# endernewton/tf-faster-rcnn

Measured on NVIDIA H100. Metric: images/sec, higher is better.
Workload: dtype f16x3 (fp32-grade: fp16 hi/lo split of both operands, 3 wgmma f16 MMAs per product, fp32 accumulate)

## Files before the change

### include/frcnn_b200.h

```cpp
#ifndef FRCNN_B200_H_
#define FRCNN_B200_H_

#include <stddef.h>
#include <stdint.h>

#ifdef __cplusplus
extern "C" {
#endif

typedef enum {
  FRCNN_OK = 0,
  FRCNN_ERR_CUDA = -1,
  FRCNN_ERR_ARG = -2,
  FRCNN_ERR_NO_DEVICE = -3,
  FRCNN_ERR_DRIVER_ENTRY = -4,
  FRCNN_ERR_CAPACITY = -5
} frcnn_status;

#define FRCNN_NMS_PLUS_ONE 1u
#define FRCNN_NMS_INCLUSIVE 2u
#define FRCNN_NMS_SKIP_DEGENERATE 4u
#define FRCNN_NMS_MODE_CPU_NMS (FRCNN_NMS_PLUS_ONE | FRCNN_NMS_INCLUSIVE)
#define FRCNN_NMS_MODE_GPU_NMS (FRCNN_NMS_PLUS_ONE)
#define FRCNN_NMS_MODE_TF (FRCNN_NMS_SKIP_DEGENERATE)

#define FRCNN_ACT_NONE 0
#define FRCNN_ACT_RELU 1
#define FRCNN_ACT_RELU6 2

int frcnn_version(void);
int frcnn_last_error(char* buf, size_t buflen);
int frcnn_check_device(int device_id);
int frcnn_zero_async(void* dev_ptr, size_t bytes, void* stream);

typedef struct frcnn_graph frcnn_graph;
int frcnn_graph_begin(void* stream);
int frcnn_graph_end(void* stream, frcnn_graph** out);
int frcnn_graph_launch(const frcnn_graph* g, void* stream);
void frcnn_graph_destroy(frcnn_graph* g);

int frcnn_nms_host(int* keep_out, int* num_out, const float* boxes_host, int boxes_num, int boxes_dim,
                   float nms_overlap_thresh, int device_id, unsigned flags);

int frcnn_nms_sorted_dev(const float* boxes_dev, int n, float thresh, unsigned flags, int max_out,
                         int* keep_dev, int* num_dev, void* stream);

typedef struct frcnn_conv_plan frcnn_conv_plan;
#define FRCNN_CONV_F16X3 0
#define FRCNN_CONV_TF32X3 1
#define FRCNN_CONV_F16X1 2

typedef struct {
  const float* in_dev;
  const void* w_hi_dev;
  const void* w_lo_dev;
  const float* scale_dev;
  const float* shift_dev;
  const float* residual_dev;
  float* out_dev;
  int n, h, w, cin;
  int cout, kh, kw, stride;
  int pad_t, pad_l;
  int ho, wo;
  int act;
  int block_n;
  int kb_per_chunk;
  int split_k;
  int impl;
  float out_mult;
  const float* in2_dev;
  int cin2;
  float* mean_dev;
  int mean_hw;
} frcnn_conv_desc;

int frcnn_conv_plan_create(frcnn_conv_plan** out, const frcnn_conv_desc* d);
int frcnn_conv_plan_run(const frcnn_conv_plan* p, void* stream);
int frcnn_conv_plan_geometry(const frcnn_conv_desc* d, int sm_count, int* out16);
int frcnn_conv_plan_info(const frcnn_conv_plan* p, int* block_n, int* tile_n, int* tile_h, int* tile_w,
                         int* grid_m, int* grid_n, int* splits, int* smem_bytes);
int frcnn_conv_plan_set_trace(frcnn_conv_plan* p, long long* trace_dev);
void frcnn_conv_plan_destroy(frcnn_conv_plan* p);
int frcnn_debug_watchdog(unsigned int* out16, int reset);

int frcnn_pack_conv_weights(const float* w_hwio_dev, void* w_hi_dev, void* w_lo_dev, int kh, int kw,
                            int cin, int cout, int wexp, void* stream);
int frcnn_pack_conv_weights_tf32(const float* w_hwio_dev, float* w_hi_dev, float* w_lo_dev, int kh, int kw,
                                 int cin, int cout, void* stream);

int frcnn_conv_first(const float* in_dev, const float* w_hwio_dev, const float* scale_dev,
                     const float* shift_dev, float* out_dev, int n, int h, int w, int cout, int k,
                     int stride, int pad_t, int pad_l, int ho, int wo, int act, void* stream);
int frcnn_depthwise3x3(const float* in_dev, const float* w_dev, const float* scale_dev,
                       const float* shift_dev, float* out_dev, int n, int h, int w, int c, int stride,
                       int pad_t, int pad_l, int ho, int wo, int act, void* stream);
int frcnn_max_pool(const float* in_dev, float* out_dev, int n, int h, int w, int c, int k, int stride,
                   int pad_t, int pad_l, int ho, int wo, int pad_is_neg_inf, void* stream);
int frcnn_spatial_mean(const float* in_dev, float* out_dev, int r, int hw, int c, void* stream);

int frcnn_preprocess(const unsigned char* img_dev, int h0, int w0, const double* means3, double fx, double fy,
                     float* blob_dev, int H, int W, void* stream);
int frcnn_preprocess_hflip(const unsigned char* img_dev, int h0, int w0, const double* means3, double fx, double fy,
                           float* blob_dev, int H, int W, void* stream);


int frcnn_rpn_decode(const float* rpn_out_dev, int ld, int delta_col, const float* base_anchors_dev, int num_anchors,
                     int batch, int fh, int fw, int feat_stride, float im_h, float im_w, float* scores_dev,
                     float* props_dev, void* stream);
size_t frcnn_sort_workspace_bytes(int n);
int frcnn_sort_desc(const float* keys_dev, int n, int batch, int* order_dev, float* sorted_keys_dev, void* workspace_dev,
                    size_t workspace_bytes, void* stream);
int frcnn_proposals(const float* props_dev, const float* scores_dev, const int* order_dev, int n, int batch,
                    int pre_nms_top_n, int post_nms_top_n, float thresh, unsigned flags, float* rois_dev,
                    float* roi_scores_dev, int* keep_dev, int* num_dev, void* stream);
int frcnn_crop_pool(const float* feat_dev, int batch, int fh, int fw, int c, const float* rois_dev, int r, int pooled,
                    int pre_pool, float* out_dev, void* stream);
#define FRCNN_ROI_ALIGN_MAX_SAMPLING 16
int frcnn_roi_align(const float* feat_dev, int batch, int fh, int fw, int c, const float* rois_dev, int r, int pooled,
                    float spatial_scale, int sampling_ratio, int aligned, float* out_dev, void* stream);
int frcnn_roi_pool(const float* feat_dev, int batch, int fh, int fw, int c, const float* rois_dev, int r, int pooled,
                   float spatial_scale, float* out_dev, void* stream);
int frcnn_cls_finish(const float* head_out_dev, int ld, int r, int num_classes, const float* stds4,
                     const float* means4, float* cls_score_dev, float* cls_prob_dev, float* bbox_pred_dev,
                     void* stream);
int frcnn_bbox_decode(const float* rois_dev, const float* bbox_pred_dev, int r, int num_classes, int batch,
                      const float* im_meta_dev, float* pred_boxes_dev, void* stream);
size_t frcnn_detect_post_workspace_bytes(int r, int num_classes, int batch);
int frcnn_detect_post(const float* cls_prob_dev, const float* pred_boxes_dev, const int* num_rois_dev, int r, int batch,
                      int num_classes, float score_thresh, float nms_thresh, unsigned flags,
                      int max_per_image, int max_det, float* det_dev, int* ndet_dev, int record_stride, int* keep_dev,
                      int* keep_cnt_dev, float* keep_score_dev, void* workspace_dev, size_t workspace_bytes, void* stream);
#define FRCNN_SOFT_NMS_LINEAR 0
#define FRCNN_SOFT_NMS_GAUSSIAN 1
#define FRCNN_SOFT_NMS_HARD 2
int frcnn_soft_nms_host(float* dets_out, int* keep_out, int* num_out, const float* dets_host, int n, int dim, int method,
                        float sigma, float nt, float score_thresh, int device_id);
int frcnn_detect_post_soft(const float* cls_prob_dev, const float* pred_boxes_dev, const int* num_rois_dev, int r, int batch,
                           int num_classes, float score_thresh, int method, float sigma, float nt, float prune_thresh,
                           int max_per_image, int max_det, float* det_dev, int* ndet_dev, int record_stride, int* keep_dev,
                           int* keep_cnt_dev, float* keep_score_dev, void* workspace_dev, size_t workspace_bytes, void* stream);
#define FRCNN_BOX_VOTE_ID 0
#define FRCNN_BOX_VOTE_AVG 1
#define FRCNN_BOX_VOTE_IOU_AVG 2
#define FRCNN_BOX_VOTE_GENERALIZED_AVG 3
#define FRCNN_BOX_VOTE_QUASI_SUM 4
#define FRCNN_BOX_VOTE_TEMP_AVG 5
int frcnn_box_vote_host(float* dets_out, const float* top_host, int n_top, int top_dim, const float* all_host, int n_all,
                        int all_dim, float thresh, int method, float beta, int device_id);
int frcnn_detect_post_vote(const float* cls_prob_dev, const float* pred_boxes_dev, const int* num_rois_dev, int r, int batch,
                           int num_classes, float score_thresh, float nms_thresh, unsigned flags, int max_per_image, int max_det,
                           float* det_dev, int* ndet_dev, int record_stride, int* keep_dev, int* keep_cnt_dev, float* keep_score_dev,
                           void* workspace_dev, size_t workspace_bytes, float vote_thresh, int vote_method, float vote_beta,
                           float* vote_box_dev, void* stream);
int frcnn_detect_post_soft_vote(const float* cls_prob_dev, const float* pred_boxes_dev, const int* num_rois_dev, int r, int batch,
                                int num_classes, float score_thresh, int method, float sigma, float nt, float prune_thresh,
                                int max_per_image, int max_det, float* det_dev, int* ndet_dev, int record_stride, int* keep_dev,
                                int* keep_cnt_dev, float* keep_score_dev, void* workspace_dev, size_t workspace_bytes,
                                float vote_thresh, int vote_method, float vote_beta, float* vote_box_dev, void* stream);
int frcnn_detect_features(const int* keep_dev, const int* keep_cnt_dev, const float* fc7_dev, int r, int batch, int num_classes,
                          int feat_dim, int max_det, float* feat_out_dev, int* roi_out_dev, void* stream);
int frcnn_detect_regions_workspace_bytes(int r, int num_classes, int batch, size_t* bytes);
// ... 19 lines not shown
```

### tf_faster_rcnn_b200/_native.py

```python
import ctypes as C
import os

_HERE = os.path.dirname(os.path.abspath(__file__))
LIB_PATH = os.path.join(_HERE, "libfrcnn_b200_wd.so" if os.environ.get("FRCNN_LIB_VARIANT") == "wd" else "libfrcnn_b200.so")

NMS_PLUS_ONE, NMS_INCLUSIVE, NMS_SKIP_DEGENERATE = 1, 2, 4
NMS_MODE_CPU_NMS = NMS_PLUS_ONE | NMS_INCLUSIVE
NMS_MODE_GPU_NMS = NMS_PLUS_ONE
NMS_MODE_TF = NMS_SKIP_DEGENERATE
ACT_NONE, ACT_RELU, ACT_RELU6 = 0, 1, 2
CONV_F16X3, CONV_TF32X3, CONV_F16X1 = 0, 1, 2
SOFT_NMS_METHODS = {"linear": 0, "gaussian": 1, "hard": 2}
AUG_MAX_VIEWS = 16
BOX_VOTE_METHODS = {"ID": 0, "AVG": 1, "IOU_AVG": 2, "GENERALIZED_AVG": 3, "QUASI_SUM": 4, "TEMP_AVG": 5}
ROI_ALIGN_MAX_SAMPLING = 16
ROI_MAX_POOLED = 16

vp, ci, cf, cu, sz = C.c_void_p, C.c_int, C.c_float, C.c_uint, C.c_size_t
ip, fp = C.POINTER(C.c_int), C.POINTER(C.c_float)


class ConvDesc(C.Structure):
    _fields_ = [("in_dev", vp), ("w_hi_dev", vp), ("w_lo_dev", vp), ("scale_dev", vp), ("shift_dev", vp),
                ("residual_dev", vp), ("out_dev", vp),
                ("n", ci), ("h", ci), ("w", ci), ("cin", ci), ("cout", ci), ("kh", ci), ("kw", ci), ("stride", ci),
                ("pad_t", ci), ("pad_l", ci), ("ho", ci), ("wo", ci), ("act", ci), ("block_n", ci), ("kb_per_chunk", ci), ("split_k", ci),
                ("impl", ci), ("out_mult", cf), ("in2_dev", vp), ("cin2", ci), ("mean_dev", vp), ("mean_hw", ci)]


SIGNATURES = {
    "frcnn_version": (ci, []),
    "frcnn_last_error": (ci, [C.c_char_p, sz]),
    "frcnn_check_device": (ci, [ci]),
    "frcnn_zero_async": (ci, [vp, sz, vp]),
    "frcnn_graph_begin": (ci, [vp]),
    "frcnn_graph_end": (ci, [vp, C.POINTER(vp)]),
    "frcnn_graph_launch": (ci, [vp, vp]),
    "frcnn_graph_destroy": (None, [vp]),
    "frcnn_nms_host": (ci, [ip, ip, fp, ci, ci, cf, ci, cu]),
    "frcnn_nms_sorted_dev": (ci, [vp, ci, cf, cu, ci, vp, vp, vp]),
    "frcnn_conv_plan_create": (ci, [C.POINTER(vp), C.POINTER(ConvDesc)]),
    "frcnn_conv_plan_run": (ci, [vp, vp]),
    "frcnn_conv_plan_geometry": (ci, [C.POINTER(ConvDesc), ci, ip]),
    "frcnn_conv_plan_info": (ci, [vp, ip, ip, ip, ip, ip, ip, ip, ip]),
    "frcnn_conv_plan_set_trace": (ci, [vp, vp]),
    "frcnn_conv_plan_destroy": (None, [vp]),
    "frcnn_debug_watchdog": (ci, [C.POINTER(C.c_uint), ci]),
    "frcnn_pack_conv_weights": (ci, [vp, vp, vp, ci, ci, ci, ci, ci, vp]),
    "frcnn_pack_conv_weights_tf32": (ci, [vp, vp, vp, ci, ci, ci, ci, vp]),
    "frcnn_conv_first": (ci, [vp, vp, vp, vp, vp, ci, ci, ci, ci, ci, ci, ci, ci, ci, ci, ci, vp]),
    "frcnn_depthwise3x3": (ci, [vp, vp, vp, vp, vp, ci, ci, ci, ci, ci, ci, ci, ci, ci, ci, vp]),
    "frcnn_max_pool": (ci, [vp, vp, ci, ci, ci, ci, ci, ci, ci, ci, ci, ci, ci, vp]),
    "frcnn_spatial_mean": (ci, [vp, vp, ci, ci, ci, vp]),
    "frcnn_preprocess": (ci, [vp, ci, ci, C.POINTER(C.c_double), C.c_double, C.c_double, vp, ci, ci, vp]),
    "frcnn_rpn_decode": (ci, [vp, ci, ci, vp, ci, ci, ci, ci, ci, cf, cf, vp, vp, vp]),
    "frcnn_sort_workspace_bytes": (sz, [ci]),
    "frcnn_sort_desc": (ci, [vp, ci, ci, vp, vp, vp, sz, vp]),
    "frcnn_proposals": (ci, [vp, vp, vp, ci, ci, ci, ci, cf, cu, vp, vp, vp, vp, vp]),
    "frcnn_crop_pool": (ci, [vp, ci, ci, ci, ci, vp, ci, ci, ci, vp, vp]),
    "frcnn_roi_align": (ci, [vp, ci, ci, ci, ci, vp, ci, ci, cf, ci, ci, vp, vp]),
    "frcnn_roi_pool": (ci, [vp, ci, ci, ci, ci, vp, ci, ci, cf, vp, vp]),
    "frcnn_cls_finish": (ci, [vp, ci, ci, ci, fp, fp, vp, vp, vp, vp]),
    "frcnn_bbox_decode": (ci, [vp, vp, ci, ci, ci, vp, vp, vp]),
    "frcnn_detect_post_workspace_bytes": (sz, [ci, ci, ci]),
    "frcnn_detect_regions_workspace_bytes": (ci, [ci, ci, ci, C.POINTER(sz)]),
    "frcnn_detect_post": (ci, [vp, vp, vp, ci, ci, ci, cf, cf, cu, ci, ci, vp, vp, ci, vp, vp, vp, vp, sz, vp]),
    "frcnn_soft_nms_host": (ci, [fp, ip, ip, fp, ci, ci, ci, cf, cf, cf, ci]),
    "frcnn_detect_post_soft": (ci, [vp, vp, vp, ci, ci, ci, cf, ci, cf, cf, cf, ci, ci, vp, vp, ci, vp, vp, vp, vp, sz, vp]),
    "frcnn_detect_features": (ci, [vp, vp, vp, ci, ci, ci, ci, ci, vp, vp, vp]),
    "frcnn_detect_regions": (ci, [vp, vp, vp, vp, vp, ci, ci, ci, ci, cf, cu, cf, ci, ci, vp, vp, vp, vp, sz, vp, vp, vp, vp, vp, vp, vp,
                                  vp, vp]),
    "frcnn_boxes_to_rois": (ci, [vp, vp, vp, ci, ci, vp, vp, vp]),
    "frcnn_preprocess_hflip": (ci, [vp, ci, ci, C.POINTER(C.c_double), C.c_double, C.c_double, vp, ci, ci, vp]),
    "frcnn_aug_union": (ci, [C.POINTER(vp), C.POINTER(vp), C.POINTER(vp), ip, ip, ci, ci, ci, vp, vp, vp, vp, vp]),
    "frcnn_box_vote_host": (ci, [fp, fp, ci, ci, fp, ci, ci, cf, ci, cf, ci]),
    "frcnn_detect_post_vote": (ci, [vp, vp, vp, ci, ci, ci, cf, cf, cu, ci, ci, vp, vp, ci, vp, vp, vp, vp, sz, cf, ci, cf, vp, vp]),
    "frcnn_detect_post_soft_vote": (ci, [vp, vp, vp, ci, ci, ci, cf, ci, cf, cf, cf, ci, ci, vp, vp, ci, vp, vp, vp, vp, sz, cf, ci, cf, vp,
                                         vp]),
}

_lib = None


def lib():
    global _lib
    if _lib is None:
        if not os.path.exists(LIB_PATH):
            raise RuntimeError("libfrcnn_b200.so not built (%s): the CUDA extension is mandatory, "
                               "there is no CPU fallback" % LIB_PATH)
        L = C.CDLL(LIB_PATH)
        for name, (res, args) in SIGNATURES.items():
            fn = getattr(L, name)
            fn.restype = res
            fn.argtypes = args
        _lib = L
    return _lib


def last_error():
    buf = C.create_string_buffer(512)
    lib().frcnn_last_error(buf, 512)
    return buf.value.decode("utf-8", "replace")


def check(rc, what=""):
    if rc != 0:
        raise RuntimeError("frcnn_b200 %s failed (status %d): %s" % (what, rc, last_error()))
```

### tf_faster_rcnn_b200/csrc/conv_gemm.cu

```cuda
#include <cuda_fp16.h>
#include "common.cuh"
#include "../../include/frcnn_b200.h"
#include <stdlib.h>
#include <string.h>

namespace frcnn {

constexpr int BLOCK_M = 128;
constexpr int BLOCK_K = 32;
constexpr int A_TILE_BYTES = BLOCK_M * BLOCK_K * 4;
constexpr int NUM_CONSUMERS = 256;
constexpr int NUM_THREADS = NUM_CONSUMERS + 128;
constexpr int REGS_PRODUCER = 40, REGS_CONSUMER = 232;
constexpr int STAGES = 3;

struct ConvKernelParams {
  float* out;
  const float* residual;
  const float* scale;
  const float* shift;
  int cout, ho, wo, nimg;
  int tn, th, tw;
  int tiles_h, tiles_w;
  int kh, kw, cin, stride, pad_t, pad_l;
  int act;
  int a_box_bytes;
  int kb_per_split;
  int m_tiles, n_tiles, total_units, n_full, splits;
  int raster_n;
  float* ws;
  long long* trace;
  int num_kb_total;
  int cin2;
  float* mean_out;
  float* mean_ws;
  int mean_hw, mean_segs, mean_ld;
};

#ifdef FRCNN_WATCHDOG
#define FRCNN_TRACE(slot, kbv)                                                              \
  do {                                                                                      \
    if (p.trace && blockIdx.x == 0 && (kbv) < 64) p.trace[(kbv) * 8 + (slot)] = clock64(); \
  } while (0)
#else
#define FRCNN_TRACE(slot, kbv) do { } while (0)
#endif

template <int MODE> struct KTraits {
  static constexpr bool TF32 = MODE == FRCNN_CONV_TF32X3;
  static constexpr bool X1 = MODE == FRCNN_CONV_F16X1;
  static constexpr int BOXES = TF32 ? 1 : 2;
  static constexpr int A_BYTES = BOXES * A_TILE_BYTES;
  static constexpr float LO_SCALE = TF32 ? 1.f : 0.00048828125f;
};
template <int BN> constexpr int b_plane_bytes() { return BN * 128; }
template <int BN, int MODE> constexpr int stage_bytes() { return KTraits<MODE>::A_BYTES + 2 * b_plane_bytes<BN>(); }
template <int BN, int MODE> constexpr int smem_bytes() {
  return STAGES * stage_bytes<BN, MODE>() + 1024  + 64 ;
}
constexpr int MEAN_COLS = 64, MEAN_LD = MEAN_COLS + 2;
constexpr int MEAN_SMEM = BLOCK_M * MEAN_LD * 4;
static_assert(smem_bytes<128, FRCNN_CONV_F16X3>() + MEAN_SMEM <= 227 * 1024, "ring exceeds the sm_90 shared-memory limit per block");

struct Unit {
  int w0, h0, n0, nblk, z, kb0, num_kb, slot;
};
__device__ __forceinline__ Unit decode_unit(const ConvKernelParams& p, int u, int num_kb_total) {
  Unit t;
  int tile;
  if (u < p.n_full) { tile = u; t.z = 0; t.slot = -1; }
  else { const int v = u - p.n_full; t.slot = v / p.splits; t.z = v - t.slot * p.splits; tile = p.n_full + t.slot; }
  int mt;
  if (p.raster_n) { t.nblk = tile % p.n_tiles; mt = tile / p.n_tiles; }
  else { mt = tile % p.m_tiles; t.nblk = tile / p.m_tiles; }
  const int tile_w = mt % p.tiles_w;
  const int tile_h = (mt / p.tiles_w) % p.tiles_h;
  const int tile_n = mt / (p.tiles_w * p.tiles_h);
  t.w0 = tile_w * p.tw; t.h0 = tile_h * p.th; t.n0 = tile_n * p.tn;
  if (t.slot < 0) { t.kb0 = 0; t.num_kb = num_kb_total; }
  else { t.kb0 = t.z * p.kb_per_split; t.num_kb = min(p.kb_per_split, num_kb_total - t.kb0); }
  return t;
}

template <int ACT>
__device__ __forceinline__ float apply_act(float a) {
  if (ACT == FRCNN_ACT_RELU) return fmaxf(a, 0.f);
  if (ACT == FRCNN_ACT_RELU6) return fminf(fmaxf(a, 0.f), 6.f);
  return a;
}

template <bool RES, int ACT>
__device__ __forceinline__ float2 finish2(const float2 v, const float2 sc, const float2 sh, const float2 r) {
  float2 y;
  y.x = __fadd_rn(__fmul_rn(v.x, sc.x), sh.x); y.y = __fadd_rn(__fmul_rn(v.y, sc.y), sh.y);
  if (RES) { y.x = __fadd_rn(y.x, r.x); y.y = __fadd_rn(y.y, r.y); }
  y.x = apply_act<ACT>(y.x); y.y = apply_act<ACT>(y.y);
  return y;
}

constexpr int EPI_CHUNK = 8;
template <int BN, bool RES, int ACT>
__device__ __forceinline__ void epilogue_vec(const ConvKernelParams& p, const float (&acc)[BN / 2], const int cbase,
                                             const int pix0, const int pix1) {
  const int cout = p.cout;
  constexpr int NJ = BN / 8;
  constexpr int CH = NJ < EPI_CHUNK ? NJ : EPI_CHUNK;
  static_assert(NJ % CH == 0, "chunking");
  const float* const res0 = RES ? p.residual + (size_t)(pix0 >= 0 ? pix0 : 0) * cout : nullptr;
  const float* const res1 = RES ? p.residual + (size_t)(pix1 >= 0 ? pix1 : 0) * cout : nullptr;
#pragma unroll
  for (int j0 = 0; j0 < NJ; j0 += CH) {
    if (cbase + 8 * j0 >= cout) break;
    float2 sc[CH], sh[CH], r0[CH], r1[CH];
#pragma unroll
    for (int jj = 0; jj < CH; ++jj) {
      const int c = cbase + 8 * (j0 + jj);
      sc[jj] = ld_nc_f2_pinned(p.scale + c);
      sh[jj] = ld_nc_f2_pinned(p.shift + c);
      if (RES) {
        r0[jj] = ld_nc_f2_pinned_if(res0 + c, pix0 >= 0 && c < cout);
        r1[jj] = ld_nc_f2_pinned_if(res1 + c, pix1 >= 0 && c < cout);
      } else {
        r0[jj] = r1[jj] = sc[jj];
      }
    }
#pragma unroll
    for (int jj = 0; jj < CH; ++jj) {
      const int j = j0 + jj;
      const int c = cbase + 8 * j;
      if (c >= cout) break;
      if (pix0 >= 0)
        *reinterpret_cast<float2*>(p.out + (size_t)pix0 * cout + c) =
            finish2<RES, ACT>(make_float2(acc[4 * j], acc[4 * j + 1]), sc[jj], sh[jj], r0[jj]);
      if (pix1 >= 0)
        *reinterpret_cast<float2*>(p.out + (size_t)pix1 * cout + c) =
            finish2<RES, ACT>(make_float2(acc[4 * j + 2], acc[4 * j + 3]), sc[jj], sh[jj], r1[jj]);
    }
  }
}

template <int BN>
__device__ __forceinline__ void epilogue_generic(const ConvKernelParams& p, const float (&acc)[BN / 2], const int cbase,
                                                 const int pix0, const int pix1) {
#pragma unroll
  for (int j = 0; j < BN / 8; ++j) {
#pragma unroll
    for (int e = 0; e < 4; ++e) {
      const int c = cbase + 8 * j + (e & 1);
      const int pix = e < 2 ? pix0 : pix1;
      if (pix < 0 || c >= p.cout) continue;
      float a = __fadd_rn(__fmul_rn(acc[4 * j + e], p.scale[c]), p.shift[c]);
      if (p.residual) a = __fadd_rn(a, __ldg(p.residual + (size_t)pix * p.cout + c));
      if (p.act == FRCNN_ACT_RELU) a = fmaxf(a, 0.f);
      else if (p.act == FRCNN_ACT_RELU6) a = fminf(fmaxf(a, 0.f), 6.f);
      p.out[(size_t)pix * p.cout + c] = a;
    }
  }
}

template <int BN, bool RES>
__device__ __forceinline__ void epilogue_dispatch(const ConvKernelParams& p, const float (&acc)[BN / 2], const int cbase,
                                                  const int pix0, const int pix1) {
  if (p.act == FRCNN_ACT_RELU) epilogue_vec<BN, RES, FRCNN_ACT_RELU>(p, acc, cbase, pix0, pix1);
  else if (p.act == FRCNN_ACT_RELU6) epilogue_vec<BN, RES, FRCNN_ACT_RELU6>(p, acc, cbase, pix0, pix1);
// ... 59 lines not shown
      float a0 = b[rs * MEAN_LD], a1 = 0.f, a2 = 0.f, a3 = 0.f;
      int r = rs + 1;
      for (; r + 3 < re; r += 4) {
        a1 = __fadd_rn(a1, b[r * MEAN_LD]); a2 = __fadd_rn(a2, b[(r + 1) * MEAN_LD]);
        a3 = __fadd_rn(a3, b[(r + 2) * MEAN_LD]); a0 = __fadd_rn(a0, b[(r + 3) * MEAN_LD]);
      }
      for (; r < re; ++r) a1 = __fadd_rn(a1, b[r * MEAN_LD]);
      p.mean_ws[((size_t)mt * p.mean_segs + s) * ld + (size_t)t.nblk * BN + cc + col] = __fadd_rn(__fadd_rn(a0, a1), __fadd_rn(a2, a3));
    }
  }
}

template <int BN>
__device__ __forceinline__ void epilogue_tile(const ConvKernelParams& p, const Unit& t, const float (&acc)[BN / 2], int r0, int q4,
                                              float* mean_buf) {
  if (p.mean_out) {
    epilogue_mean<BN>(p, t, acc, r0, q4, mean_buf);
    return;
  }
  if (t.slot >= 0) {
    float* const w = p.ws + ((size_t)t.slot * p.splits + t.z) * (size_t)(BLOCK_M * BN) + 2 * q4;
#pragma unroll
    for (int j = 0; j < BN / 8; ++j) {
      __stcg(reinterpret_cast<float2*>(w + (size_t)r0 * BN + 8 * j), make_float2(acc[4 * j], acc[4 * j + 1]));
      __stcg(reinterpret_cast<float2*>(w + (size_t)(r0 + 8) * BN + 8 * j), make_float2(acc[4 * j + 2], acc[4 * j + 3]));
    }
    return;
  }
  const int pix0 = tile_pixel(p, t, r0), pix1 = tile_pixel(p, t, r0 + 8);
  const int cbase = t.nblk * BN + 2 * q4;
  if ((p.cout & 3) != 0) {
    epilogue_generic<BN>(p, acc, cbase, pix0, pix1);
    return;
  }
  if (p.residual) epilogue_dispatch<BN, true>(p, acc, cbase, pix0, pix1);
  else epilogue_dispatch<BN, false>(p, acc, cbase, pix0, pix1);
}

template <int BN, int MODE>
__device__ __forceinline__ void wgmma_rs(float (&d)[BN / 2], const uint32_t (&a)[4], uint64_t b_desc, uint32_t scale_d) {
  if (KTraits<MODE>::TF32) wgmma_tf32_rs<BN>(d, a, b_desc, scale_d);
  else wgmma_f16_rs<BN>(d, a, b_desc, scale_d);
}

template <int BN, int MODE>
__global__ void __launch_bounds__(NUM_THREADS, 1)
conv_gemm_kernel(const __grid_constant__ CUtensorMap tmA, const __grid_constant__ CUtensorMap tmA2,
                 const __grid_constant__ CUtensorMap tmBhi, const __grid_constant__ CUtensorMap tmBlo, const ConvKernelParams p) {
  using T = KTraits<MODE>;
  constexpr int kStage = stage_bytes<BN, MODE>();
  constexpr int kPlane = b_plane_bytes<BN>();
  constexpr int NACC = BN / 2;
  static_assert(BN == 64 || BN == 128, "block_n");

  extern __shared__ uint8_t smem_raw[];
  uint8_t* smem = reinterpret_cast<uint8_t*>((reinterpret_cast<uintptr_t>(smem_raw) + 1023) & ~uintptr_t(1023));
  uint64_t* full = reinterpret_cast<uint64_t*>(smem + STAGES * kStage);
  uint64_t* empty = full + STAGES;

  const int warp = threadIdx.x >> 5;
  const int lane = threadIdx.x & 31;
  const int num_kb_total = p.num_kb_total;

  if (threadIdx.x == NUM_CONSUMERS) {
    tma_prefetch_desc(&tmA); tma_prefetch_desc(&tmBhi); tma_prefetch_desc(&tmBlo);
    if (p.cin2) tma_prefetch_desc(&tmA2);
    for (int s = 0; s < STAGES; ++s) { mbar_init(&full[s], 1); mbar_init(&empty[s], NUM_CONSUMERS); }
    mbar_fence_init();
  }
  __syncthreads();
  pdl_launch_dependents();
  pdl_wait();

  if (warp >= NUM_CONSUMERS / 32) {
    reg_dec<REGS_PRODUCER>();
    if (warp == NUM_CONSUMERS / 32 && lane == 0) {
      const int cchunks = p.cin / BLOCK_K;
      const int total1 = p.kh * p.kw * cchunks;
      const int cchunks2 = p.cin2 / BLOCK_K;
      const uint32_t tx = (uint32_t)(T::BOXES * p.a_box_bytes + (T::X1 ? 1 : 2) * kPlane);
      int s = 0; uint32_t ph = 0, kbt = 0;
      for (int u = blockIdx.x; u < p.total_units; u += gridDim.x) {
        const Unit t = decode_unit(p, u, num_kb_total);
#pragma unroll 1
        for (int kb = 0; kb < t.num_kb; ++kb, ++kbt) {
          MBAR_WAIT(&empty[s], ph ^ 1u, 4, kbt);
          uint8_t* st = smem + s * kStage;
          mbar_expect_tx(&full[s], tx);
#pragma unroll
          for (int i = 0; i < T::BOXES; ++i) {
            const int g32 = (t.kb0 + kb) * T::BOXES + i;
            int tap = g32 / cchunks, kc = g32 - tap * cchunks;
            const CUtensorMap* ma = &tmA;
            if (g32 >= total1) {
              tap = 0;
              if (cchunks2) { ma = &tmA2; kc = min(g32 - total1, cchunks2); }
              else kc = cchunks;
            }
            const int r = tap / p.kw, sx = tap - r * p.kw;
            tma_load_4d(st + i * A_TILE_BYTES, ma, &full[s], kc * BLOCK_K, t.w0 * p.stride + sx - p.pad_l,
                        t.h0 * p.stride + r - p.pad_t, t.n0);
          }
          const int kcoord = (t.kb0 + kb) * T::BOXES * BLOCK_K;
          tma_load_2d(st + T::A_BYTES, &tmBhi, &full[s], kcoord, t.nblk * BN);
          if (!T::X1) tma_load_2d(st + T::A_BYTES + kPlane, &tmBlo, &full[s], kcoord, t.nblk * BN);
          FRCNN_TRACE(0, kbt);
          if (++s == STAGES) { s = 0; ph ^= 1u; }
        }
      }
    }
    return;
  }

  reg_inc<REGS_CONSUMER>();
  const int wg = warp >> 2;
  const int q4 = lane & 3;
  const int r0 = wg * 64 + (warp & 3) * 16 + (lane >> 2);
  const uint32_t swz = (uint32_t)(lane >> 2);
  uint32_t aoff[4][2];
#pragma unroll
  for (int j = 0; j < 4; ++j)
#pragma unroll
    for (int h = 0; h < 2; ++h) {
      const int ch = T::TF32 ? j * 8 + h * 4 + q4 : (j & 1) * 16 + h * 8 + 2 * q4;
      const int box = T::TF32 ? 0 : j >> 1;
      aoff[j][h] = (uint32_t)(box * A_TILE_BYTES + r0 * 128) + ((((uint32_t)ch >> 2) ^ swz) << 4) + (((uint32_t)ch & 3u) << 2);
    }
  const uint32_t smem0 = smem_u32(smem);
  int s = 0; uint32_t ph = 0, kbt = 0;
  for (int u = blockIdx.x; u < p.total_units; u += gridDim.x) {
    const Unit t = decode_unit(p, u, num_kb_total);
    float acc[NACC], part[NACC];
#pragma unroll
    for (int i = 0; i < NACC; ++i) { acc[i] = 0.f; part[i] = 0.f; }
#pragma unroll 1
    for (int kb = 0; kb < t.num_kb; ++kb, ++kbt) {
      MBAR_WAIT(&full[s], ph, 1, kbt);
      if (threadIdx.x == 0) FRCNN_TRACE(1, kbt);
      const uint32_t sa = smem0 + (uint32_t)(s * kStage);
      uint32_t ahi[4][4], alo[4][4];
#pragma unroll
      for (int j = 0; j < 4; ++j) {
#pragma unroll
        for (int f = 0; f < 4; ++f) {
          const uint32_t addr = sa + aoff[j][f >> 1] + ((f & 1) ? 1024u : 0u);
          if (T::TF32) {
            float x;
            asm volatile("ld.shared.f32 %0, [%1];" : "=f"(x) : "r"(addr));
            const float hi = to_tf32(x);
            ahi[j][f] = __float_as_uint(hi);
            alo[j][f] = __float_as_uint(to_tf32_fast(__fsub_rn(x, hi)));
          } else {
            float2 x;
            asm volatile("ld.shared.v2.f32 {%0, %1}, [%2];" : "=f"(x.x), "=f"(x.y) : "r"(addr));
            const uint32_t h = pack_f16x2_rn(x.x, x.y);
            const float2 fh = __half22float2(*reinterpret_cast<const __half2*>(&h));
            ahi[j][f] = h;
            alo[j][f] = T::X1 ? 0u : pack_f16x2_rn(__fmul_rn(__fsub_rn(x.x, fh.x), 2048.f), __fmul_rn(__fsub_rn(x.y, fh.y), 2048.f));
          }
        }
      }
      const uint64_t bhi = wgmma_sw128_desc(sa + (uint32_t)T::A_BYTES);
      const uint64_t blo = wgmma_sw128_desc(sa + (uint32_t)(T::A_BYTES + kPlane));
#pragma unroll
      for (int i = 0; i < NACC; ++i) reg_fence(part[i]);
      wgmma_fence();
#pragma unroll
      for (int j = 0; j < 4; ++j) wgmma_rs<BN, MODE>(part, ahi[j], bhi + 2u * j, j > 0 ? 1u : 0u);
      wgmma_commit();
      wgmma_wait_all();
#pragma unroll
      for (int i = 0; i < NACC; ++i) { reg_fence(part[i]); acc[i] = __fadd_rn(acc[i], part[i]); }
      if (!T::X1) {
        wgmma_fence();
#pragma unroll
        for (int j = 0; j < 4; ++j) {
          wgmma_rs<BN, MODE>(part, alo[j], bhi + 2u * j, j > 0 ? 1u : 0u);
          wgmma_rs<BN, MODE>(part, ahi[j], blo + 2u * j, 1u);
        }
        wgmma_commit();
        wgmma_wait_all();
#pragma unroll
        for (int i = 0; i < NACC; ++i) { reg_fence(part[i]); acc[i] = __fmaf_rn(part[i], T::LO_SCALE, acc[i]); }
      }
      mbar_arrive(&empty[s]);
      if (threadIdx.x == 0) FRCNN_TRACE(2, kbt);
      if (++s == STAGES) { s = 0; ph ^= 1u; }
    }
    epilogue_tile<BN>(p, t, acc, r0, q4, reinterpret_cast<float*>(full + 8));
  }
}

template <int BN>
__global__ void __launch_bounds__(256)
tail_reduce_kernel(const ConvKernelParams p) {
  pdl_launch_dependents();
  pdl_wait();
  constexpr int RPB = 256 / (BN / 4);
  constexpr int GROUPS = BLOCK_M / RPB;
  const int slot = blockIdx.x / GROUPS, rgroup = blockIdx.x % GROUPS;
  const int tile = p.n_full + slot;
  const int mt = p.raster_n ? tile / p.n_tiles : tile % p.m_tiles, nblk = p.raster_n ? tile % p.n_tiles : tile / p.m_tiles;
  const int tile_w = mt % p.tiles_w, tile_h = (mt / p.tiles_w) % p.tiles_h, tile_n = mt / (p.tiles_w * p.tiles_h);
  const int rows_img = p.th * p.tw;
  constexpr int C4 = BN / 4;
  static_assert(256 % C4 == 0, "each thread keeps one fixed channel group");
  const float* base = p.ws + (size_t)slot * p.splits * (size_t)(BLOCK_M * BN);
  const bool vec_ok = (p.cout & 3) == 0;
  const int cg = threadIdx.x % C4;
  const int c = nblk * BN + cg * 4;
  if (c >= p.cout) return;
  const float4 sc4 = __ldg(reinterpret_cast<const float4*>(p.scale + c)), sh4 = __ldg(reinterpret_cast<const float4*>(p.shift + c));
  const float sc[4] = {sc4.x, sc4.y, sc4.z, sc4.w}, sh[4] = {sh4.x, sh4.y, sh4.z, sh4.w};
  {
    const int row = rgroup * RPB + threadIdx.x / C4;
    const int dn = row / rows_img, rem = row % rows_img;
    const int n = tile_n * p.tn + dn, h = tile_h * p.th + rem / p.tw, w = tile_w * p.tw + rem % p.tw;
    if (row >= p.tn * rows_img || n >= p.nimg || h >= p.ho || w >= p.wo) return;
    const size_t o = ((((size_t)n * p.ho + h) * p.wo + w)) * p.cout + c;
// ... 94 lines not shown
using namespace frcnn;

struct frcnn_conv_plan {
  CUtensorMap tmA, tmA2, tmBhi, tmBlo;
  ConvKernelParams kp;
  int block_n, stages, smem;
  int impl;
  dim3 grid;
  int n_tail;
  float* ws;
  float* eff;
  float* mean_ws;
};

static void choose_tile(int n, int ho, int wo, int stride, int* tn, int* th, int* tw) {
  long best_tiles = -1; int bn = 1, bh = 1, bw = 1; int best_rows = 0;
  const int lim = 256 / stride;
  for (int a = 1; a <= n && a <= BLOCK_M; ++a)
    for (int b = 1; b <= ho && a * b <= BLOCK_M && b <= lim; ++b) {
      int c = BLOCK_M / (a * b);
      if (c > wo) c = wo;
      if (c > lim) c = lim;
      if (c < 1) continue;
      int tiles_w = cdiv(wo, c);
      c = cdiv(wo, tiles_w);
      long tiles = (long)cdiv(n, a) * cdiv(ho, b) * tiles_w;
      int rows = a * b * c;
      if (best_tiles < 0 || tiles < best_tiles || (tiles == best_tiles && rows < best_rows)) {
        best_tiles = tiles; bn = a; bh = b; bw = c; best_rows = rows;
      }
    }
  *tn = bn; *th = bh; *tw = bw;
}

static bool pdl_enabled() {
  static int v = -1;
  if (v < 0) { const char* e = getenv("FRCNN_NO_PDL"); v = (e && e[0] == '1') ? 0 : 1; }
  return v == 1;
}

template <int BN, int MODE>
static int launch(const frcnn_conv_plan* p, cudaStream_t st) {
  static bool attr_done = false;
  if (!attr_done) {
    FRCNN_CUDA(cudaFuncSetAttribute(conv_gemm_kernel<BN, MODE>, cudaFuncAttributeMaxDynamicSharedMemorySize,
                                    smem_bytes<BN, MODE>() + MEAN_SMEM));
    attr_done = true;
  }
  cudaLaunchAttribute attr[1];
  attr[0].id = cudaLaunchAttributeProgrammaticStreamSerialization;
  attr[0].val.programmaticStreamSerializationAllowed = 1;
  const bool pdl = pdl_enabled();
  cudaLaunchConfig_t cfg{};
  cfg.gridDim = p->grid; cfg.blockDim = dim3(NUM_THREADS); cfg.stream = st;
  cfg.dynamicSmemBytes = smem_bytes<BN, MODE>() + (p->kp.mean_out ? MEAN_SMEM : 0);
  cfg.attrs = attr; cfg.numAttrs = pdl ? 1 : 0;
  FRCNN_CUDA(cudaLaunchKernelEx(&cfg, conv_gemm_kernel<BN, MODE>, p->tmA, p->tmA2, p->tmBhi, p->tmBlo, p->kp));
  if (p->kp.mean_out) {
    cudaLaunchConfig_t mc{};
    const long n = (long)(p->kp.wo / p->kp.mean_hw) * p->kp.cout;
    mc.gridDim = dim3((unsigned)((n + 255) / 256)); mc.blockDim = dim3(256); mc.dynamicSmemBytes = 0; mc.stream = st;
    mc.attrs = attr; mc.numAttrs = pdl ? 1 : 0;
    FRCNN_CUDA(cudaLaunchKernelEx(&mc, mean_finish_kernel, p->kp));
  }
  if (p->n_tail > 0) {
    cudaLaunchConfig_t rc{};
    rc.gridDim = dim3((unsigned)(p->n_tail * (BLOCK_M / (256 / (BN / 4))))); rc.blockDim = dim3(256); rc.dynamicSmemBytes = 0; rc.stream = st;
    rc.attrs = attr; rc.numAttrs = pdl ? 1 : 0;
    FRCNN_CUDA(cudaLaunchKernelEx(&rc, tail_reduce_kernel<BN>, p->kp));
  }
  return OK;
}

struct Geometry {
  int n, h, w, ho, wo;
  int tn, th, tw, tiles_w, tiles_h, tiles_n;
  long m_tiles;
  int num_kb, bn, n_tiles, kpc;
  long tiles, n_tail;
  int splits, kbs;
  long total_units;
  int grid;
  int raster_n;
};

static int decide_geometry(const frcnn_conv_desc* d, int sms, Geometry* g) {
  FRCNN_REQUIRE(d->cin > 0 && d->cin % BLOCK_K == 0, "cin=%d must be a positive multiple of 32", d->cin);
  FRCNN_REQUIRE(d->kh >= 1 && d->kw >= 1 && d->stride >= 1 && d->stride <= 8, "bad filter geometry");
  FRCNN_REQUIRE(d->n > 0 && d->h > 0 && d->w > 0 && d->ho > 0 && d->wo > 0 && d->cout > 0, "bad shape");
  FRCNN_REQUIRE(sms > 0, "bad SM count");
  g->n = d->n; g->h = d->h; g->w = d->w; g->ho = d->ho; g->wo = d->wo;
  const bool pointwise = d->kh == 1 && d->kw == 1 && d->stride == 1 && d->pad_t == 0 && d->pad_l == 0 && g->ho == g->h && g->wo == g->w;
  const bool mean = d->mean_hw != 0;
  FRCNN_REQUIRE(d->cin2 >= 0 && d->cin2 % BLOCK_K == 0, "cin2=%d must be 0 or a positive multiple of 32", d->cin2);
  FRCNN_REQUIRE(d->cin2 == 0 || pointwise, "a second A source needs a pointwise layer (1x1, stride 1, no padding)");
  FRCNN_REQUIRE(!mean || pointwise, "the mean epilogue needs a pointwise layer (1x1, stride 1, no padding)");
  FRCNN_REQUIRE(!mean || d->cout % 4 == 0, "the mean epilogue needs cout %% 4 == 0 (cout=%d)", d->cout);
  FRCNN_REQUIRE(d->mean_hw >= 0 && (!mean || ((long)d->n * d->h * d->w) % d->mean_hw == 0),
                "mean_hw=%d must be positive and divide the pixel count", d->mean_hw);
  FRCNN_REQUIRE(!mean || d->split_k <= 1, "the mean epilogue is never split along K");
  if (pointwise) {
    g->w = g->wo = g->n * g->h * g->w; g->n = 1; g->h = g->ho = 1;
  }
  const int ktot = d->kh * d->kw * d->cin + d->cin2;
  choose_tile(g->n, g->ho, g->wo, d->stride, &g->tn, &g->th, &g->tw);
  g->tiles_w = cdiv(g->wo, g->tw); g->tiles_h = cdiv(g->ho, g->th); g->tiles_n = cdiv(g->n, g->tn);
  g->m_tiles = (long)g->tiles_w * g->tiles_h * g->tiles_n;
  const bool f16 = d->impl != FRCNN_CONV_TF32X3;
  const int ks = f16 ? 2 : 1;
  g->num_kb = cdiv(ktot / BLOCK_K, ks);
  g->kpc = d->kb_per_chunk > 0 ? d->kb_per_chunk : 8 / ks;
  int bn = d->block_n;
  if (bn == 0) {
    long best = -1;
    const int cands[2] = {128, 64};
    for (int i = 0; i < 2; ++i) {
      const int c = cands[i];
      if (c > 64 && c / 2 >= d->cout) continue;
      const long ctas = g->m_tiles * cdiv(d->cout, c);
      const long waves = (ctas + sms - 1) / sms;
      const long cost = f16 ? waves * (g->num_kb * 900L + 4000L) : waves * (g->num_kb * 1400L + 6000L);
      if (best < 0 || cost < best) { best = cost; bn = c; }
    }
  }
  FRCNN_REQUIRE(bn == 64 || bn == 128, "block_n must be 64 or 128");
  g->bn = bn;
  g->n_tiles = cdiv(d->cout, bn);
  g->tiles = g->m_tiles * g->n_tiles;
  FRCNN_REQUIRE(g->tiles <= 0x3fffffffL, "too many tiles");
  long n_tail = 0; int splits = 1;
  const int num_kb = g->num_kb;
  const int max_split = num_kb * ks / 8 < 8 ? num_kb * ks / 8 : 8;
  if (d->split_k > 1) {
    n_tail = g->tiles; splits = d->split_k;
  } else if (d->split_k == 0 && max_split >= 2) {
    const long rem = g->tiles % sms;
    if (g->tiles <= sms / 2) { if (num_kb * ks >= 16) { n_tail = g->tiles; splits = (int)(sms / g->tiles); } }
    else if (g->tiles > sms && rem > 0 && rem <= sms / 2 && num_kb * ks >= 48) { n_tail = rem; splits = (int)(sms / rem); }
    if (splits > max_split) splits = max_split;
    if (splits < 2) { n_tail = 0; splits = 1; }
  }
  int kbs = cdiv(num_kb, splits);
  splits = cdiv(num_kb, kbs);
  if (splits < 2 || (d->cout & 3) != 0 || mean) { n_tail = 0; splits = 1; kbs = num_kb; }
  FRCNN_REQUIRE(splits <= 64, "bad split_k");
  g->n_tail = n_tail; g->splits = splits; g->kbs = kbs;
  g->total_units = (g->tiles - n_tail) + n_tail * splits;
  FRCNN_REQUIRE(g->total_units <= 0x7fffffffL, "too many work units");
  g->grid = (int)(g->total_units < sms ? g->total_units : sms);
  {
    const char* e = getenv("FRCNN_CONV_RASTER");
    const double a_bytes = (double)d->n * d->h * d->w * (d->cin + d->cin2) * 4.0, b_bytes = (double)d->cout * ktot * 4.0;
    g->raster_n = (e && (e[0] == 'm' || e[0] == 'n')) ? (e[0] == 'n') : (a_bytes > b_bytes && g->n_tiles > 1);
  }
  return OK;
}

extern "C" int frcnn_conv_plan_geometry(const frcnn_conv_desc* d, int sm_count, int* out16) {
  FRCNN_REQUIRE(d && out16, "null argument");
  Geometry g;
  int rc = decide_geometry(d, sm_count, &g);
  if (rc) return rc;
  const int v[16] = {g.bn, g.tn, g.th, g.tw, (int)g.m_tiles, g.n_tiles, (int)g.tiles, (int)g.n_tail, g.splits, g.kbs,
                     (int)g.total_units, g.grid, g.num_kb, g.kpc, g.tiles_h, g.tiles_w};
  for (int i = 0; i < 16; ++i) out16[i] = v[i];
  return OK;
}

extern "C" int frcnn_conv_plan_create(frcnn_conv_plan** out, const frcnn_conv_desc* d) {
  FRCNN_REQUIRE(out && d, "null argument");
  FRCNN_REQUIRE(d->in_dev && d->w_hi_dev && d->w_lo_dev && (d->mean_hw ? d->mean_dev != nullptr : d->out_dev != nullptr),
                "null device pointer");
  FRCNN_REQUIRE(d->cin2 == 0 || d->in2_dev, "cin2=%d without in2_dev", d->cin2);
  int sms = 132;
  { int dev = 0; cudaDeviceProp pr; if (cudaGetDevice(&dev) == cudaSuccess && cudaGetDeviceProperties(&pr, dev) == cudaSuccess && pr.multiProcessorCount > 0) sms = pr.multiProcessorCount; }
  Geometry g;
  int grc = decide_geometry(d, sms, &g);
  if (grc) return grc;
  frcnn_conv_plan* p = (frcnn_conv_plan*)aligned_alloc(64, (sizeof(frcnn_conv_plan) + 63) / 64 * 64);
  if (!p) { set_error("out of host memory"); return ERR_ARG; }
  memset(p, 0, sizeof(*p));
  const int bn = g.bn;
  {
    uint64_t dims[4] = {(uint64_t)d->cin, (uint64_t)g.w, (uint64_t)g.h, (uint64_t)g.n};
    uint64_t strides[3] = {(uint64_t)d->cin * 4, (uint64_t)g.w * d->cin * 4, (uint64_t)g.h * g.w * d->cin * 4};
    uint32_t box[4] = {(uint32_t)BLOCK_K, (uint32_t)(g.tw * d->stride), (uint32_t)(g.th * d->stride), (uint32_t)g.tn};
    uint32_t es[4] = {1, (uint32_t)d->stride, (uint32_t)d->stride, 1};
    int rc = encode_map(&p->tmA, d->in_dev, 4, dims, strides, box, es);
    if (rc) { free(p); return rc; }
    p->tmA2 = p->tmA;
    if (d->cin2 > 0) {
      uint64_t dims2[4] = {(uint64_t)d->cin2, (uint64_t)g.w, (uint64_t)g.h, (uint64_t)g.n};
      uint64_t strides2[3] = {(uint64_t)d->cin2 * 4, (uint64_t)g.w * d->cin2 * 4, (uint64_t)g.h * g.w * d->cin2 * 4};
      rc = encode_map(&p->tmA2, d->in2_dev, 4, dims2, strides2, box, es);
      if (rc) { free(p); return rc; }
    }
  }
  const bool f16 = d->impl != FRCNN_CONV_TF32X3;
  {
    const uint64_t ktot = (uint64_t)d->kh * d->kw * d->cin + d->cin2;
    uint64_t dims[2] = {ktot, (uint64_t)d->cout};
    uint64_t strides[1] = {ktot * (f16 ? 2 : 4)};
    uint32_t box[2] = {(uint32_t)(f16 ? 2 * BLOCK_K : BLOCK_K), (uint32_t)bn};
    uint32_t es[2] = {1, 1};
    const CUtensorMapDataType dt = f16 ? CU_TENSOR_MAP_DATA_TYPE_FLOAT16 : CU_TENSOR_MAP_DATA_TYPE_FLOAT32;
    const CUtensorMapSwizzle sw = CU_TENSOR_MAP_SWIZZLE_128B;
    int rc = encode_map(&p->tmBhi, d->w_hi_dev, 2, dims, strides, box, es, dt, sw);
    if (!rc) rc = encode_map(&p->tmBlo, d->w_lo_dev, 2, dims, strides, box, es, dt, sw);
    if (rc) { free(p); return rc; }
  }
  ConvKernelParams& k = p->kp;
  k.out = d->out_dev; k.residual = d->residual_dev;
  k.cout = d->cout; k.ho = g.ho; k.wo = g.wo; k.nimg = g.n;
  k.tn = g.tn; k.th = g.th; k.tw = g.tw; k.tiles_h = g.tiles_h; k.tiles_w = g.tiles_w;
  k.kh = d->kh; k.kw = d->kw; k.cin = d->cin; k.stride = d->stride; k.pad_t = d->pad_t; k.pad_l = d->pad_l;
  k.act = d->act;
  k.a_box_bytes = g.tn * g.th * g.tw * BLOCK_K * 4;
  k.trace = nullptr;
  k.num_kb_total = g.num_kb;
  k.m_tiles = (int)g.m_tiles; k.n_tiles = g.n_tiles;
  k.kb_per_split = g.kbs; k.splits = g.splits; k.n_full = (int)(g.tiles - g.n_tail);
  k.total_units = (int)g.total_units;
  k.raster_n = g.raster_n;
  k.cin2 = d->cin2;
  k.mean_out = d->mean_hw ? d->mean_dev : nullptr; k.mean_ws = nullptr; k.mean_hw = d->mean_hw; k.mean_ld = g.n_tiles * bn;
  k.mean_segs = d->mean_hw ? (g.tw < cdiv(g.tw - 1, d->mean_hw) + 1 ? g.tw : cdiv(g.tw - 1, d->mean_hw) + 1) : 0;
  k.ws = nullptr; p->ws = nullptr; p->eff = nullptr; p->mean_ws = nullptr; p->n_tail = (int)g.n_tail;
  {
    const int padded = g.n_tiles * bn;
    const float om = f16 ? (d->out_mult != 0.f ? d->out_mult : 1.f) : 1.f;
    cudaError_t e = cudaMalloc(&p->eff, (size_t)2 * padded * sizeof(float));
    if (e != cudaSuccess) { free(p); return cuda_fail(e, "epilogue vectors", __FILE__, __LINE__); }
    prep_epilogue_vectors_kernel<<<cdiv(padded, 256), 256>>>(d->scale_dev, d->shift_dev, om, d->cout, padded, p->eff, p->eff + padded);
    e = cudaGetLastError();
    if (e == cudaSuccess) e = cudaDeviceSynchronize();
    if (e != cudaSuccess) { cudaFree(p->eff); free(p); return cuda_fail(e, "prep_epilogue_vectors", __FILE__, __LINE__); }
    k.scale = p->eff; k.shift = p->eff + padded;
  }
  if (g.n_tail > 0) {
    cudaError_t e = cudaMalloc(&p->ws, (size_t)g.n_tail * g.splits * BLOCK_M * bn * sizeof(float));
    if (e != cudaSuccess) { cudaFree(p->eff); free(p); return cuda_fail(e, "split-tile workspace", __FILE__, __LINE__); }
    k.ws = p->ws;
  }
  if (d->mean_hw) {
    cudaError_t e = cudaMalloc(&p->mean_ws, (size_t)g.m_tiles * k.mean_segs * k.mean_ld * sizeof(float));
    if (e != cudaSuccess) { cudaFree(p->eff); free(p); return cuda_fail(e, "mean workspace", __FILE__, __LINE__); }
    k.mean_ws = p->mean_ws;
  }
  p->grid = dim3((unsigned)g.grid, 1, 1);
  p->block_n = bn;
  p->impl = f16 ? (d->impl == FRCNN_CONV_F16X1 ? FRCNN_CONV_F16X1 : FRCNN_CONV_F16X3) : FRCNN_CONV_TF32X3;
  p->stages = STAGES;
  p->smem = f16 ? (bn == 128 ? smem_bytes<128, FRCNN_CONV_F16X3>() : smem_bytes<64, FRCNN_CONV_F16X3>())
              : (bn == 128 ? smem_bytes<128, FRCNN_CONV_TF32X3>() : smem_bytes<64, FRCNN_CONV_TF32X3>());
  if (d->mean_hw) p->smem += MEAN_SMEM;
  *out = p;
  return OK;
}

extern "C" int frcnn_conv_plan_run(const frcnn_conv_plan* p, void* stream) {
  FRCNN_REQUIRE(p, "null plan");
  cudaStream_t st = (cudaStream_t)stream;
  if (p->impl == FRCNN_CONV_F16X3) return p->block_n == 128 ? launch<128, FRCNN_CONV_F16X3>(p, st) : launch<64, FRCNN_CONV_F16X3>(p, st);
  if (p->impl == FRCNN_CONV_F16X1) return p->block_n == 128 ? launch<128, FRCNN_CONV_F16X1>(p, st) : launch<64, FRCNN_CONV_F16X1>(p, st);
  return p->block_n == 128 ? launch<128, FRCNN_CONV_TF32X3>(p, st) : launch<64, FRCNN_CONV_TF32X3>(p, st);
}

extern "C" int frcnn_conv_plan_info(const frcnn_conv_plan* p, int* block_n, int* tile_n, int* tile_h, int* tile_w,
                                    int* grid_m, int* grid_n, int* stages, int* smem) {
  FRCNN_REQUIRE(p, "null plan");
  if (block_n) *block_n = p->block_n;
  if (tile_n) *tile_n = p->kp.tn;
  if (tile_h) *tile_h = p->kp.th;
  if (tile_w) *tile_w = p->kp.tw;
  if (grid_m) *grid_m = p->kp.m_tiles;
  if (grid_n) *grid_n = p->kp.n_tiles;
  if (stages) *stages = p->n_tail > 0 ? p->kp.splits : 1;
  if (smem) *smem = p->smem;
  return OK;
}

extern "C" int frcnn_debug_watchdog(unsigned int* out16, int reset) {
  FRCNN_REQUIRE(out16, "null argument");
#ifdef FRCNN_WATCHDOG
  FRCNN_CUDA(cudaMemcpyFromSymbol(out16, g_watchdog, 16 * sizeof(unsigned int)));
  if (reset) { unsigned int z[16] = {0}; FRCNN_CUDA(cudaMemcpyToSymbol(g_watchdog, z, sizeof(z))); }
  return OK;
#else
  (void)reset;
  for (int i = 0; i < 16; ++i) out16[i] = 0;
  out16[15] = 0xffffffffu;
  return OK;
#endif
}

extern "C" int frcnn_conv_plan_set_trace(frcnn_conv_plan* p, long long* trace_dev) {
  FRCNN_REQUIRE(p, "null plan");
  p->kp.trace = trace_dev;
  return OK;
}

extern "C" void frcnn_conv_plan_destroy(frcnn_conv_plan* p) {
  if (p && p->ws) cudaFree(p->ws);
  if (p && p->eff) cudaFree(p->eff);
  if (p && p->mean_ws) cudaFree(p->mean_ws);
  free(p);
}
// ... 1 lines not shown
```

Measured before the change: 259.4.

## Skip K-blocks whose filter taps read only padding for a tile

```diff
diff --git a/include/frcnn_b200.h b/include/frcnn_b200.h
--- a/include/frcnn_b200.h
+++ b/include/frcnn_b200.h
@@ -77,6 +77,7 @@
 int frcnn_conv_plan_create(frcnn_conv_plan** out, const frcnn_conv_desc* d);
 int frcnn_conv_plan_run(const frcnn_conv_plan* p, void* stream);
 int frcnn_conv_plan_geometry(const frcnn_conv_desc* d, int sm_count, int* out16);
+int frcnn_conv_plan_live_kblocks(const frcnn_conv_desc* d, int sm_count, long long* total);
 int frcnn_conv_plan_info(const frcnn_conv_plan* p, int* block_n, int* tile_n, int* tile_h, int* tile_w,
                          int* grid_m, int* grid_n, int* splits, int* smem_bytes);
 int frcnn_conv_plan_set_trace(frcnn_conv_plan* p, long long* trace_dev);
diff --git a/tf_faster_rcnn_b200/_native.py b/tf_faster_rcnn_b200/_native.py
--- a/tf_faster_rcnn_b200/_native.py
+++ b/tf_faster_rcnn_b200/_native.py
@@ -42,6 +42,7 @@
     "frcnn_conv_plan_create": (ci, [C.POINTER(vp), C.POINTER(ConvDesc)]),
     "frcnn_conv_plan_run": (ci, [vp, vp]),
     "frcnn_conv_plan_geometry": (ci, [C.POINTER(ConvDesc), ci, ip]),
+    "frcnn_conv_plan_live_kblocks": (ci, [C.POINTER(ConvDesc), ci, C.POINTER(C.c_longlong)]),
     "frcnn_conv_plan_info": (ci, [vp, ip, ip, ip, ip, ip, ip, ip, ip]),
     "frcnn_conv_plan_set_trace": (ci, [vp, vp]),
     "frcnn_conv_plan_destroy": (None, [vp]),
diff --git a/tf_faster_rcnn_b200/csrc/conv_gemm.cu b/tf_faster_rcnn_b200/csrc/conv_gemm.cu
--- a/tf_faster_rcnn_b200/csrc/conv_gemm.cu
+++ b/tf_faster_rcnn_b200/csrc/conv_gemm.cu
@@ -31,6 +31,8 @@
   float* ws;
   long long* trace;
   int num_kb_total;
+  int kb_per_tap;
+  int h, w;
   int cin2;
   float* mean_out;
   float* mean_ws;
@@ -65,7 +67,7 @@
 struct Unit {
   int w0, h0, n0, nblk, z, kb0, num_kb, slot;
 };
-__device__ __forceinline__ Unit decode_unit(const ConvKernelParams& p, int u, int num_kb_total) {
+__host__ __device__ __forceinline__ Unit decode_unit(const ConvKernelParams& p, int u, int num_kb_total) {
   Unit t;
   int tile;
   if (u < p.n_full) { tile = u; t.z = 0; t.slot = -1; }
@@ -78,8 +80,52 @@
   const int tile_n = mt / (p.tiles_w * p.tiles_h);
   t.w0 = tile_w * p.tw; t.h0 = tile_h * p.th; t.n0 = tile_n * p.tn;
   if (t.slot < 0) { t.kb0 = 0; t.num_kb = num_kb_total; }
-  else { t.kb0 = t.z * p.kb_per_split; t.num_kb = min(p.kb_per_split, num_kb_total - t.kb0); }
+  else { t.kb0 = t.z * p.kb_per_split; t.num_kb = p.kb_per_split < num_kb_total - t.kb0 ? p.kb_per_split : num_kb_total - t.kb0; }
   return t;
+}
+
+struct LiveKb {
+  int r_lo, r_hi, row_kb, col_begin, col_end;
+};
+
+__host__ __device__ __forceinline__ void live_span(int o0, int k, int pad, int stride, int n_out, int in, int* lo, int* hi) {
+  *lo = 0; *hi = -1;
+#pragma unroll 1
+  for (int r = k - 1; r >= 0; --r) {
+    const int base = o0 * stride + r - pad;
+    const int i0 = base >= 0 ? 0 : (-base + stride - 1) / stride;
+    if (i0 < n_out && base + stride * i0 < in) { *lo = r; if (*hi < 0) *hi = r; }
+  }
+}
+
+__host__ __device__ __forceinline__ LiveKb live_kblocks(const ConvKernelParams& p, const Unit& t) {
+  LiveKb L;
+  if (p.kb_per_tap == 0) { L.r_lo = 0; L.r_hi = 0; L.row_kb = 0; L.col_begin = 0; L.col_end = p.num_kb_total; return L; }
+  int s_lo, s_hi;
+  live_span(t.h0, p.kh, p.pad_t, p.stride, p.th, p.h, &L.r_lo, &L.r_hi);
+  live_span(t.w0, p.kw, p.pad_l, p.stride, p.tw, p.w, &s_lo, &s_hi);
+  if (s_lo > s_hi) L.r_hi = L.r_lo - 1;
+  L.row_kb = p.kw * p.kb_per_tap;
+  L.col_begin = s_lo * p.kb_per_tap;
+  L.col_end = (s_hi + 1) * p.kb_per_tap;
+  return L;
+}
+
+__host__ __device__ __forceinline__ void live_row(const LiveKb& L, int r, int kb0, int kb1, int* b, int* e) {
+  const int rb = r * L.row_kb + L.col_begin, re = r * L.row_kb + L.col_end;
+  *b = rb > kb0 ? rb : kb0;
+  *e = re < kb1 ? re : kb1;
+}
+
+__host__ __device__ __forceinline__ int live_kb_count(const LiveKb& L, int kb0, int kb1) {
+  int n = 0;
+#pragma unroll 1
+  for (int r = L.r_lo; r <= L.r_hi; ++r) {
+    int b, e;
+    live_row(L, r, kb0, kb1, &b, &e);
+    if (e > b) n += e - b;
+  }
+  return n;
 }
 
 template <int ACT>
@@ -305,30 +351,36 @@
       int s = 0; uint32_t ph = 0, kbt = 0;
       for (int u = blockIdx.x; u < p.total_units; u += gridDim.x) {
         const Unit t = decode_unit(p, u, num_kb_total);
+        const LiveKb L = live_kblocks(p, t);
 #pragma unroll 1
-        for (int kb = 0; kb < t.num_kb; ++kb, ++kbt) {
-          MBAR_WAIT(&empty[s], ph ^ 1u, 4, kbt);
-          uint8_t* st = smem + s * kStage;
-          mbar_expect_tx(&full[s], tx);
-#pragma unroll
-          for (int i = 0; i < T::BOXES; ++i) {
-            const int g32 = (t.kb0 + kb) * T::BOXES + i;
-            int tap = g32 / cchunks, kc = g32 - tap * cchunks;
-            const CUtensorMap* ma = &tmA;
-            if (g32 >= total1) {
-              tap = 0;
-              if (cchunks2) { ma = &tmA2; kc = min(g32 - total1, cchunks2); }
-              else kc = cchunks;
+        for (int lr = L.r_lo; lr <= L.r_hi; ++lr) {
+          int kb_begin, kb_end;
+          live_row(L, lr, t.kb0, t.kb0 + t.num_kb, &kb_begin, &kb_end);
+#pragma unroll 1
+          for (int kb = kb_begin; kb < kb_end; ++kb, ++kbt) {
+            MBAR_WAIT(&empty[s], ph ^ 1u, 4, kbt);
+            uint8_t* st = smem + s * kStage;
+            mbar_expect_tx(&full[s], tx);
+#pragma unroll
+            for (int i = 0; i < T::BOXES; ++i) {
+              const int g32 = kb * T::BOXES + i;
+              int tap = g32 / cchunks, kc = g32 - tap * cchunks;
+              const CUtensorMap* ma = &tmA;
+              if (g32 >= total1) {
+                tap = 0;
+                if (cchunks2) { ma = &tmA2; kc = min(g32 - total1, cchunks2); }
+                else kc = cchunks;
+              }
+              const int r = tap / p.kw, sx = tap - r * p.kw;
+              tma_load_4d(st + i * A_TILE_BYTES, ma, &full[s], kc * BLOCK_K, t.w0 * p.stride + sx - p.pad_l,
+                          t.h0 * p.stride + r - p.pad_t, t.n0);
             }
-            const int r = tap / p.kw, sx = tap - r * p.kw;
-            tma_load_4d(st + i * A_TILE_BYTES, ma, &full[s], kc * BLOCK_K, t.w0 * p.stride + sx - p.pad_l,
-                        t.h0 * p.stride + r - p.pad_t, t.n0);
+            const int kcoord = kb * T::BOXES * BLOCK_K;
+            tma_load_2d(st + T::A_BYTES, &tmBhi, &full[s], kcoord, t.nblk * BN);
+            if (!T::X1) tma_load_2d(st + T::A_BYTES + kPlane, &tmBlo, &full[s], kcoord, t.nblk * BN);
+            FRCNN_TRACE(0, kbt);
+            if (++s == STAGES) { s = 0; ph ^= 1u; }
           }
-          const int kcoord = (t.kb0 + kb) * T::BOXES * BLOCK_K;
-          tma_load_2d(st + T::A_BYTES, &tmBhi, &full[s], kcoord, t.nblk * BN);
-          if (!T::X1) tma_load_2d(st + T::A_BYTES + kPlane, &tmBlo, &full[s], kcoord, t.nblk * BN);
-          FRCNN_TRACE(0, kbt);
-          if (++s == STAGES) { s = 0; ph ^= 1u; }
         }
       }
     }
@@ -353,11 +405,12 @@
   int s = 0; uint32_t ph = 0, kbt = 0;
   for (int u = blockIdx.x; u < p.total_units; u += gridDim.x) {
     const Unit t = decode_unit(p, u, num_kb_total);
+    const int num_kb = live_kb_count(live_kblocks(p, t), t.kb0, t.kb0 + t.num_kb);
     float acc[NACC], part[NACC];
 #pragma unroll
     for (int i = 0; i < NACC; ++i) { acc[i] = 0.f; part[i] = 0.f; }
 #pragma unroll 1
-    for (int kb = 0; kb < t.num_kb; ++kb, ++kbt) {
+    for (int kb = 0; kb < num_kb; ++kb, ++kbt) {
       MBAR_WAIT(&full[s], ph, 1, kbt);
       if (threadIdx.x == 0) FRCNN_TRACE(1, kbt);
       const uint32_t sa = smem0 + (uint32_t)(s * kStage);
@@ -618,6 +671,7 @@
   long total_units;
   int grid;
   int raster_n;
+  int kb_per_tap;
 };
 
 static int decide_geometry(const frcnn_conv_desc* d, int sms, Geometry* g) {
@@ -646,6 +700,7 @@
   const int ks = f16 ? 2 : 1;
   g->num_kb = cdiv(ktot / BLOCK_K, ks);
   g->kpc = d->kb_per_chunk > 0 ? d->kb_per_chunk : 8 / ks;
+  g->kb_per_tap = (d->cin2 == 0 && d->cin % (ks * BLOCK_K) == 0) ? d->cin / (ks * BLOCK_K) : 0;
   int bn = d->block_n;
   if (bn == 0) {
     long best = -1;
@@ -700,6 +755,44 @@
   const int v[16] = {g.bn, g.tn, g.th, g.tw, (int)g.m_tiles, g.n_tiles, (int)g.tiles, (int)g.n_tail, g.splits, g.kbs,
                      (int)g.total_units, g.grid, g.num_kb, g.kpc, g.tiles_h, g.tiles_w};
   for (int i = 0; i < 16; ++i) out16[i] = v[i];
+  return OK;
+}
+
+static long long issued_kblocks(const ConvKernelParams& k) {
+  long long n = 0;
+  for (int u = 0; u < k.total_units; ++u) {
+    const Unit t = decode_unit(k, u, k.num_kb_total);
+    n += live_kb_count(live_kblocks(k, t), t.kb0, t.kb0 + t.num_kb);
+  }
+  return n;
+}
+
+static void geometry_params(const frcnn_conv_desc* d, const Geometry& g, ConvKernelParams* k) {
+  k->cout = d->cout; k->ho = g.ho; k->wo = g.wo; k->nimg = g.n;
+  k->tn = g.tn; k->th = g.th; k->tw = g.tw; k->tiles_h = g.tiles_h; k->tiles_w = g.tiles_w;
+  k->kh = d->kh; k->kw = d->kw; k->cin = d->cin; k->stride = d->stride; k->pad_t = d->pad_t; k->pad_l = d->pad_l;
+  k->act = d->act;
+  k->a_box_bytes = g.tn * g.th * g.tw * BLOCK_K * 4;
+  k->num_kb_total = g.num_kb;
+  k->kb_per_tap = g.kb_per_tap;
+  k->h = g.h; k->w = g.w;
+  k->m_tiles = (int)g.m_tiles; k->n_tiles = g.n_tiles;
+  k->kb_per_split = g.kbs; k->splits = g.splits; k->n_full = (int)(g.tiles - g.n_tail);
+  k->total_units = (int)g.total_units;
+  k->raster_n = g.raster_n;
+  k->cin2 = d->cin2;
+  if (k->kb_per_tap && issued_kblocks(*k) == (long long)g.tiles * g.num_kb) k->kb_per_tap = 0;
+}
+
+extern "C" int frcnn_conv_plan_live_kblocks(const frcnn_conv_desc* d, int sm_count, long long* total) {
+  FRCNN_REQUIRE(d && total, "null argument");
+  Geometry g;
+  int rc = decide_geometry(d, sm_count, &g);
+  if (rc) return rc;
+  ConvKernelParams k;
+  memset(&k, 0, sizeof(k));
+  geometry_params(d, g, &k);
+  *total = issued_kblocks(k);
   return OK;
 }
 
@@ -746,19 +839,9 @@
     if (rc) { free(p); return rc; }
   }
   ConvKernelParams& k = p->kp;
+  geometry_params(d, g, &k);
   k.out = d->out_dev; k.residual = d->residual_dev;
-  k.cout = d->cout; k.ho = g.ho; k.wo = g.wo; k.nimg = g.n;
-  k.tn = g.tn; k.th = g.th; k.tw = g.tw; k.tiles_h = g.tiles_h; k.tiles_w = g.tiles_w;
-  k.kh = d->kh; k.kw = d->kw; k.cin = d->cin; k.stride = d->stride; k.pad_t = d->pad_t; k.pad_l = d->pad_l;
-  k.act = d->act;
-  k.a_box_bytes = g.tn * g.th * g.tw * BLOCK_K * 4;
   k.trace = nullptr;
-  k.num_kb_total = g.num_kb;
-  k.m_tiles = (int)g.m_tiles; k.n_tiles = g.n_tiles;
-  k.kb_per_split = g.kbs; k.splits = g.splits; k.n_full = (int)(g.tiles - g.n_tail);
-  k.total_units = (int)g.total_units;
-  k.raster_n = g.raster_n;
-  k.cin2 = d->cin2;
   k.mean_out = d->mean_hw ? d->mean_dev : nullptr; k.mean_ws = nullptr; k.mean_hw = d->mean_hw; k.mean_ld = g.n_tiles * bn;
   k.mean_segs = d->mean_hw ? (g.tw < cdiv(g.tw - 1, d->mean_hw) + 1 ? g.tw : cdiv(g.tw - 1, d->mean_hw) + 1) : 0;
   k.ws = nullptr; p->ws = nullptr; p->eff = nullptr; p->mean_ws = nullptr; p->n_tail = (int)g.n_tail;
```

New measurement: 263.0 (median of 6 runs). 1.01x the previous value.
